# MinghanLi/UniVS

Hardware: AMD Instinct MI355X
Metric: frames/sec per node, 720p T=5 clip, Swin-T 100Q; mask-logit max-abs-err (higher is better)
Workload: dtype f32; 1 GPU; BASELINE config 2: Swin-T UniVS, T=5 @ 720p (736x1280 padded), 100 queries, first clip (no prompt queries); one clip per GPU; frames_per_clip=5, queries=100, parallelism=clip-replicas x1

## Files before the change

univs_amd/build.py:

```python
import os
import shutil
import subprocess
import sys

HERE = os.path.dirname(os.path.abspath(__file__))
CSRC = os.path.join(HERE, "csrc")
LIB = os.path.join(HERE, "libunivs_hip.so")
SOURCES = ["capi.hip", "msda_fwd.hip", "msda_tiled2.hip", "msda_strips.hip", "msda_heads.hip", "msda_bwd.hip", "msda_prepare.hip", "mask_decode.hip", "linear_split.hip", "linear_f16x3.hip", "linear_pair_f16x3.hip", "linear_pair_xres.hip", "gemm_f16x3_stream.hip", "gemm_f16x3_tile.hip", "mlp_f16x3.hip", "small_linear.hip", "cross_attn.hip", "window_attn.hip", "window_attn_f16.hip", "window_attn_qkv.hip", "resample.hip", "semantic_extract.hip", "layer_norm.hip", "group_norm.hip", "softmax.hip", "proca_attn.hip", "prompt_sampler.hip", "transpose.hip", "mask_stats.hip", "image_post.hip", "video_post.hip", "pair_count.hip", "vss_count.hip", "davis_count.hip", "vis_overlap.hip", "pvos_count.hip", "semantic_decode.hip", "frame_resize.hip", "mask_prompt_resize.hip", "png_deflate.hip"]
HEADERS = [os.path.join(CSRC, "common.h"), os.path.join(CSRC, "msda_common.h"), os.path.join(CSRC, "msda_geometry.h"), os.path.join(CSRC, "msda_dev.h"), os.path.join(CSRC, "msda_window_geom.h"), os.path.join(CSRC, "msda_strips_geom.h"), os.path.join(CSRC, "msda_heads_geom.h"), os.path.join(CSRC, "config.h"), os.path.join(CSRC, "window_attn.h"), os.path.join(CSRC, "f16x3.h"), os.path.join(CSRC, "f16x3_kstep.h"), os.path.join(CSRC, "gemm_plan.h"), os.path.join(CSRC, "pair_xres_plan.h"), os.path.join(CSRC, "resample_taps.h"),
           os.path.join(CSRC, "mask_post.h"), os.path.join(CSRC, "count_core.h"), os.path.join(CSRC, "launchers.h"), os.path.join(CSRC, "xattn_merge.h"), os.path.join(CSRC, "skinny_gemm_f32.h"), os.path.join(HERE, "..", "include", "univs_hip.h"),
           os.path.join(HERE, "..", "include", "univs_eval_hip.h"), os.path.join(HERE, "..", "include", "univs_fused_hip.h"),
           os.path.join(HERE, "..", "include", "univs_pvos_hip.h"), os.path.join(HERE, "..", "include", "univs_semantic_hip.h"),
           os.path.join(HERE, "..", "include", "univs_encoder_hip.h"), os.path.join(HERE, "..", "include", "univs_swin_hip.h"),
           os.path.join(HERE, "..", "include", "univs_frames_hip.h"), os.path.join(HERE, "..", "include", "univs_prompts_hip.h"),
           os.path.join(HERE, "..", "include", "univs_png_hip.h")]


def _hipcc():
    for c in (os.environ.get("HIPCC"), shutil.which("hipcc"), "/opt/rocm/bin/hipcc"):
        if c and os.path.exists(c):
            return c
    raise RuntimeError("hipcc not found (set HIPCC or install ROCm)")


def needs_build():
    if not os.path.exists(LIB):
        return True
    t = os.path.getmtime(LIB)
    deps = [os.path.join(CSRC, s) for s in SOURCES if os.path.exists(os.path.join(CSRC, s))] + HEADERS
    return any(os.path.getmtime(d) > t for d in deps)


def _flags(defines=()):
    return ["--offload-arch=gfx950", "-O3", "-std=c++17", "-fPIC", "-fno-gpu-rdc", "-Wall", "-Wno-unused-function",
            "-I", os.path.join(HERE, "..", "include"), *[f"-D{d}" for d in defines]]


def build(force=False, verbose=True, lib=LIB, defines=(), tag=""):
    if not force and not defines and not needs_build():
        return lib
    from concurrent.futures import ThreadPoolExecutor
    objdir = os.path.join(HERE, "_obj" + tag)
    os.makedirs(objdir, exist_ok=True)
    hipcc = _hipcc()
    hdr_t = max(os.path.getmtime(h) for h in HEADERS)
    srcs = [s for s in SOURCES if os.path.exists(os.path.join(CSRC, s))]

    def compile_one(s):
        src, obj = os.path.join(CSRC, s), os.path.join(objdir, s.replace(".hip", ".o"))
        if not force and os.path.exists(obj) and os.path.getmtime(obj) > max(os.path.getmtime(src), hdr_t):
            return obj
        cmd = [hipcc, *_flags(defines), "-c", src, "-o", obj]
        if verbose:
            print("[univs_amd.build]", " ".join(cmd), file=sys.stderr, flush=True)
        subprocess.run(cmd, check=True)
        return obj

    with ThreadPoolExecutor(max_workers=min(8, os.cpu_count() or 2)) as ex:
        objs = list(ex.map(compile_one, srcs))
    cmd = [hipcc, "--offload-arch=gfx950", "-fPIC", "-shared", "-fno-gpu-rdc", *objs, "-o", lib + ".tmp"]
    if verbose:
        print("[univs_amd.build]", " ".join(cmd), file=sys.stderr, flush=True)
    subprocess.run(cmd, check=True)
    os.replace(lib + ".tmp", lib)
    return lib


ABLATIONS = {"plainsplit": ("UNIVS_SPLIT_PLAIN",), "nosplit": ("UNIVS_ABLATE_NOSPLIT",), "nomfma": ("UNIVS_ABLATE_NOMFMA",),
             "nosplit_nomfma": ("UNIVS_ABLATE_NOSPLIT", "UNIVS_ABLATE_NOMFMA"), "trace": ("UNIVS_TRACE_GEMM",), "vtpad8": ("UNIVS_WH_VT_PAD=8", "UNIVS_XA_VS=40"), "gs256": ("UNIVS_GS_THREADS=256",),
             "trace_nosplit_nomfma": ("UNIVS_TRACE_GEMM", "UNIVS_ABLATE_NOSPLIT", "UNIVS_ABLATE_NOMFMA"),
             "heads_nostream": ("S6_ABLATE=1",), "heads_norows": ("S6_ABLATE=2",), "heads_noreduce": ("S6_ABLATE=4",),
             "heads_norecords": ("S6_ABLATE=8",), "heads_nostream_norows": ("S6_ABLATE=3",), "heads_onlyrows": ("S6_ABLATE=13",),
             "heads_skeleton": ("S6_ABLATE=15",), "heads_trace": ("S6_TRACE",),
             "mlp_regstage": ("UNIVS_MLP_REGSTAGE",), "mlp_trace": ("UNIVS_TRACE_MLP",),
             "mlp_trace_nomfma": ("UNIVS_TRACE_MLP", "ML_PS_ABL=1"), "mlp_trace_noreads": ("UNIVS_TRACE_MLP", "ML_PS_ABL=2")}


def build_ablation(name, verbose=False):
    lib = os.path.join(HERE, f"libunivs_hip_{name}.so")
    return build(force=False, verbose=verbose, lib=lib, defines=ABLATIONS[name], tag="_" + name)


if __name__ == "__main__":
    if "--ablate" in sys.argv:
        print(build_ablation(sys.argv[sys.argv.index("--ablate") + 1]))
    else:
        build(force="--force" in sys.argv)
        print(LIB)
```

univs_amd/csrc/gemm_f16x3_stream.hip:

```cpp
#include "common.h"
#include "config.h"
#include "f16x3_kstep.h"
#include "gemm_plan.h"
#include "launchers.h"

#include <algorithm>
#include <cstdlib>

namespace univs {

#ifdef UNIVS_TRACE_GEMM
UNIVS_GT_DECL(g_gs_trace);
#endif
enum { GS_EPI_NONE = EPI_NONE, GS_EPI_RELU = EPI_RELU, GS_EPI_GELU = EPI_GELU, GS_EPI_RESIDUAL = EPI_RESIDUAL };

__global__ __launch_bounds__(256) void presplit_f16x3_kernel(const float* __restrict__ W, int N, int K, int conv_cin, int kperm,
                                                             u32x4* __restrict__ Wp, float* __restrict__ winv) {
  __shared__ unsigned smax;
  const int r = blockIdx.x;
  if (threadIdx.x == 0) smax = 0u;
  __syncthreads();
  const float* src = W + (size_t)r * K;
  auto elem = [&](int k) __attribute__((always_inline)) -> float {
    if (conv_cin == 0) return src[k];
    const int tap = k / conv_cin, ci = k - tap * conv_cin;
    return src[ci * 9 + tap];
  };
  unsigned mx = 0u;
  for (int k = threadIdx.x; k < K; k += blockDim.x) mx = max(mx, __builtin_bit_cast(unsigned, fabsf(elem(k))));
  atomicMax(&smax, mx);
  __syncthreads();
  float s, inv;
  l3_scale(smax, 14, s, inv);
  if (threadIdx.x == 0) winv[r] = inv;
  for (int kc = threadIdx.x; kc < (K >> 3); kc += blockDim.x) {
    f32x4 v0, v1;
#pragma unroll
    for (int e = 0; e < 4; ++e) {
      const int k0 = kperm ? (kc >> 2) * 32 + 4 * (kc & 3) + e : kc * 8 + e;
      v0[e] = elem(k0);
      v1[e] = elem(kperm ? k0 + 16 : k0 + 4);
    }
    f16x8 h, m;
    l3_split8(v0, v1, s, h, m);
    Wp[(size_t)(kc * 2) * N + r] = __builtin_bit_cast(u32x4, h);
    Wp[(size_t)(kc * 2 + 1) * N + r] = __builtin_bit_cast(u32x4, m);
  }
}

int presplit_f16x3(const float* w, int N, int K, int conv_cin, int kperm, void* wp, float* winv, hipStream_t st) {
  if (N <= 0) return UNIVS_OK;
  hipLaunchKernelGGL(presplit_f16x3_kernel, dim3(N), dim3(256), 0, st, w, N, K, conv_cin, kperm, reinterpret_cast<u32x4*>(wp), winv);
  return check_launch("presplit_f16x3");
}

struct GsArgs {
  const float* X;
  const u32x4* Wp;
  const float* winv;
  const float* bias;
  const float* Res;
  float* Y;
  int M, N, K, rows_per_pass, epi;
  int Cin, Cout, H, Wd, HW;
  int tap0;
  int remap;
  const float* affine;
};

template <int RB, int RING, int XMODE, bool AFF = false>
__global__ __launch_bounds__(GS_THREADS, 512 / GS_THREADS) void gemm_f16x3_stream(const GsArgs a) {
  extern __shared__ __attribute__((aligned(16))) u32x4 Wst[];
  [[maybe_unused]] const int gts = UNIVS_GT_SLOT();
  UNIVS_GT(g_gs_trace, gts, 0);
  UNIVS_GT_REAL(g_gs_trace, gts, 62);
  constexpr int Rp = 16 * RB;
  constexpr int SLAB = RING * 4 * 2 * Rp;
  unsigned bx = blockIdx.x, by = blockIdx.y;
  if (a.remap && gridDim.y > 1) {
    const unsigned lw = xcd_remap(blockIdx.x + gridDim.x * blockIdx.y, gridDim.x * gridDim.y);
    bx = lw / gridDim.y;
    by = lw - bx * gridDim.y;
  }
  const int n0 = by * a.rows_per_pass;
  const int R = min(a.rows_per_pass, a.N - n0);
  const int tid = threadIdx.x, lane = tid & 63;
  const int wave = __builtin_amdgcn_readfirstlane(tid >> 6);
  const int M = a.M, N = a.N, K = a.K, epi = a.epi;
  const int KS = K >> 5, KG = KS / RING;
  const int j = lane & 15, g = lane >> 4;
  float* bias_lds = reinterpret_cast<float*>(Wst + 2 * SLAB);
  float* winv_lds = bias_lds + Rp;
  [[maybe_unused]] float* aff_lds = winv_lds + Rp;
  constexpr int NWV = GS_THREADS / 64;

  const int WT = (M + GS_TILE_M - 1) / GS_TILE_M;
  const int wg0 = (int)((long long)WT * bx / gridDim.x), wg1 = (int)((long long)WT * (bx + 1) / gridDim.x);
  const int rounds = (wg1 - wg0 + NWV - 1) / NWV;
  if (rounds == 0) return;

  for (int r = tid; r < Rp; r += GS_THREADS) {
    bias_lds[r] = (a.bias && r < R) ? a.bias[n0 + r] : 0.f;
    winv_lds[r] = r < R ? a.winv[n0 + r] : 0.f;
  }

  constexpr int UNITS = RING * 8 * Rp;
  constexpr int UPT = (UNITS + GS_THREADS - 1) / GS_THREADS;
  constexpr int UPS = (UPT + RING - 1) / RING;
  u32x4 wreg[UPS];
  auto w_fetch = [&](int q, int u) __attribute__((always_inline)) {
#pragma unroll
    for (int v = 0; v < UPS; ++v) {
      const int i = tid + GS_THREADS * (u * UPS + v);
      const int run = i / Rp, rr = i - run * Rp;
      wreg[v] = (u32x4){0u, 0u, 0u, 0u};
      if (u * UPS + v < UPT && i < UNITS && rr < R) wreg[v] = a.Wp[(size_t)(q * RING * 8 + run) * N + n0 + rr];
    }
  };
  auto w_commit = [&](int buf, int u) __attribute__((always_inline)) {
#pragma unroll
    for (int v = 0; v < UPS; ++v) {
      const int i = tid + GS_THREADS * (u * UPS + v);
      if (u * UPS + v < UPT && i < UNITS) Wst[buf * SLAB + i] = wreg[v];
    }
  };
#pragma unroll
  for (int u = 0; u < RING; ++u) {
    w_fetch(0, u);
    w_commit(0, u);
  }

  const long long xbytes = XMODE == 0 ? (long long)M * K * 4 : (long long)(M / a.HW) * a.Cin * a.HW * 4;
  const __amdgpu_buffer_rsrc_t xrs = __builtin_amdgcn_make_buffer_rsrc(const_cast<float*>(a.X), 0, (int)xbytes, 0x00020000);
  const long long ybytes = XMODE == 0 ? (long long)M * N * 4 : (long long)(M / a.HW) * a.Cout * a.HW * 4;
  const __amdgpu_buffer_rsrc_t yrs = __builtin_amdgcn_make_buffer_rsrc(a.Y, 0, (int)ybytes, 0x00020000);
  const __amdgpu_buffer_rsrc_t rrs =
      __builtin_amdgcn_make_buffer_rsrc(const_cast<float*>(epi == GS_EPI_RESIDUAL ? a.Res : a.X), 0, (int)ybytes, 0x00020000);

  struct TileRows {
    unsigned vo[2];
    int py[2], px[2];
    unsigned ao[2];
  };
  auto tile_rows = [&](int tt, TileRows& t) __attribute__((always_inline)) {
#pragma unroll
    for (int c = 0; c < 2; ++c) {
      const int m = min(tt * GS_TILE_M + 16 * c + j, M - 1);
      if (XMODE == 0) {
        t.vo[c] = ((unsigned)m * (unsigned)K + (unsigned)(8 * g)) * 4u;
        t.py[c] = t.px[c] = 0;
        t.ao[c] = 0u;
      } else if (XMODE == 2) {
        const int f = m / a.HW, rem = m - f * a.HW;
        t.py[c] = AFF ? 0 : rem / a.Wd;
        t.px[c] = AFF ? 0 : rem - t.py[c] * a.Wd;
        t.vo[c] = ((unsigned)m * (unsigned)a.Cin + (unsigned)(8 * g)) * 4u;
        t.ao[c] = (unsigned)(((f & 1) * a.Cin + 8 * g) * 8);
      } else {
        const int f = m / a.HW, rem = m - f * a.HW;
        t.py[c] = AFF ? 0 : rem / a.Wd;
        t.px[c] = AFF ? 0 : rem - t.py[c] * a.Wd;
        t.vo[c] = (unsigned)((f * a.Cin + 8 * g) * a.HW + rem) * 4u;
        t.ao[c] = (unsigned)(((f & 1) * a.Cin + 8 * g) * 8);
      }
    }
  };
  f32x4 raw[RING][2][2];
  const int kspt = XMODE != 0 ? a.Cin >> 5 : 1;
  auto load_x = [&](f32x4 (&buf)[2][2], const TileRows& t, int ks) __attribute__((always_inline)) {
    if (XMODE == 0) {
#pragma unroll
      for (int c = 0; c < 2; ++c) {
        buf[c][0] = __builtin_bit_cast(f32x4, __builtin_amdgcn_raw_buffer_load_b128(xrs, t.vo[c], ks * 128, 0));
        buf[c][1] = __builtin_bit_cast(f32x4, __builtin_amdgcn_raw_buffer_load_b128(xrs, t.vo[c] + 16u, ks * 128, 0));
      }
    } else if (XMODE == 2) {
      const int tap_ = ks / kspt, cb = (ks - tap_ * kspt) * 32;
      const int tap = tap_ + a.tap0;
      const int dy = tap / 3 - 1, dx = tap - (tap / 3) * 3 - 1;
#pragma unroll
      for (int c = 0; c < 2; ++c) {
        const bool inb = AFF || ((unsigned)(t.py[c] + dy) < (unsigned)a.H && (unsigned)(t.px[c] + dx) < (unsigned)a.Wd);
        const unsigned vo = inb ? t.vo[c] + (unsigned)((dy * a.Wd + dx) * a.Cin * 4) : 0xFFFFFFE0u;
        buf[c][0] = __builtin_bit_cast(f32x4, __builtin_amdgcn_raw_buffer_load_b128(xrs, vo, cb * 4, 0));
        buf[c][1] = __builtin_bit_cast(f32x4, __builtin_amdgcn_raw_buffer_load_b128(xrs, vo + 16u, cb * 4, 0));
      }
    } else {
      const int tap_ = ks / kspt, cb = (ks - tap_ * kspt) * 32;
      const int tap = tap_ + a.tap0;
      const int dy = tap / 3 - 1, dx = tap - (tap / 3) * 3 - 1;
#pragma unroll
      for (int c = 0; c < 2; ++c) {
        const bool inb = AFF || ((unsigned)(t.py[c] + dy) < (unsigned)a.H && (unsigned)(t.px[c] + dx) < (unsigned)a.Wd);
        const unsigned vo = inb ? t.vo[c] + (unsigned)((dy * a.Wd + dx) * 4) : 0xFFFFFFF0u;
#pragma unroll
        for (int e = 0; e < 8; ++e)
          buf[c][e >> 2][e & 3] = __builtin_bit_cast(float, __builtin_amdgcn_raw_buffer_load_b32(xrs, vo, (cb + e) * a.HW * 4, 0));
      }
    }
  };

  f32x4 acc[RB][2];
  int eset[2];
  float sx[2], sx_inv[2];
  using KS_ = KStep<RB>;
  constexpr int NB = KS_::NB;
  typename KS_::Batch afr[2];
  const unsigned a_lane = KS_::lane(g, j);
  auto read_batch = l3_batch_reader<RB>();

  TileRows t_cur, t_next;
  tile_rows(wg0 + wave, t_cur);
  tile_rows(wg0 + min(1, rounds - 1) * NWV + wave, t_next);
#pragma unroll
  for (int u = 0; u < RING; ++u) load_x(raw[u], t_cur, u);

  UNIVS_GT(g_gs_trace, gts, 2);
  UNIVS_GT_VAL(g_gs_trace, gts, 63, rounds);
  int gq = 0;
  [[maybe_unused]] int aff_f0 = -1, aff_f1 = -1;
#pragma unroll 1
  for (int rd = 0; rd < rounds; ++rd) {
    const int tt = wg0 + rd * NWV + wave;
    const bool tile_ok = tt < wg1;
    if constexpr (AFF) {
      const int r0 = min((wg0 + rd * NWV) * GS_TILE_M, M - 1), r1 = min(r0 + NWV * GS_TILE_M - 1, M - 1);
      const int f0 = r0 / a.HW, f1 = r1 / a.HW;
      if (f0 != aff_f0 || f1 != aff_f1) {
        __syncthreads();
        const int n = (f1 - f0 + 1) * a.Cin;
        for (int i = tid; i < n; i += GS_THREADS) {
          const int f = i < a.Cin ? f0 : f1, ch = i < a.Cin ? i : i - a.Cin;
          *reinterpret_cast<float2*>(aff_lds + ((f & 1) * a.Cin + ch) * 2) = *reinterpret_cast<const float2*>(a.affine + ((size_t)f * a.Cin + ch) * 2);
        }
        aff_f0 = f0;
        aff_f1 = f1;
      }
    }
#pragma unroll
    for (int rb = 0; rb < RB; ++rb) acc[rb][0] = acc[rb][1] = (f32x4){0.f, 0.f, 0.f, 0.f};
    l3_row_scale_reset(eset, sx, sx_inv);
#pragma unroll 1
    for (int q = 0; q < KG; ++q, ++gq) {
      __syncthreads();
      const int bufc = gq & 1, qn = (q + 1 == KG) ? 0 : q + 1;
      const bool last_group = q + 1 == KG;
      const unsigned a_buf = a_lane + (unsigned)(bufc * SLAB * 16);
      read_batch(afr[0], a_buf, std::integral_constant<int, 0>{});
#pragma unroll
      for (int u = 0; u < RING; ++u) {
        if (u > 0) w_commit(bufc ^ 1, u - 1);
        if constexpr (AFF) {
          const unsigned kb = (unsigned)((q * RING + u) * 32 * 8);
#pragma unroll
          for (int c = 0; c < 2; ++c) {
            const f32x4* ap = reinterpret_cast<const f32x4*>(reinterpret_cast<const char*>(aff_lds) + t_cur.ao[c] + kb);
#pragma unroll
            for (int h = 0; h < 2; ++h) {
              const f32x4 p0 = ap[2 * h], p1 = ap[2 * h + 1];
              raw[u][c][h][0] = fmaxf(fma_single(raw[u][c][h][0], p0[0], p0[1]), 0.f);
              raw[u][c][h][1] = fmaxf(fma_single(raw[u][c][h][1], p0[2], p0[3]), 0.f);
              raw[u][c][h][2] = fmaxf(fma_single(raw[u][c][h][2], p1[0], p1[1]), 0.f);
              raw[u][c][h][3] = fmaxf(fma_single(raw[u][c][h][3], p1[2], p1[3]), 0.f);
            }
            __builtin_amdgcn_sched_barrier(0);
          }
        }
        int enew[2];
        if (__builtin_amdgcn_ballot_w64(l3_row_scale_need(raw[u], eset, enew)) != 0) {
#pragma unroll
          for (int c = 0; c < 2; ++c) {
            const bool mine = enew[c] > eset[c] + 2;
            const int en = mine ? enew[c] : eset[c];
            const float ratio = __builtin_bit_cast(float, (unsigned)(127 + max(eset[c] - en, -126)) << 23);
#pragma unroll
            for (int rb = 0; rb < RB; ++rb) acc[rb][c] *= ratio;
            eset[c] = en;
            sx[c] = __builtin_bit_cast(float, (unsigned)(127 + 12 - en) << 23);
            sx_inv[c] = __builtin_bit_cast(float, (unsigned)(127 - 12 + en) << 23);
          }
        }
        float s0 = sx[0], s1 = sx[1];
        asm volatile("" : "+v"(s0), "+v"(s1) : : "memory");
        f16x8 bh[2], bm[2];
        l3_split8(raw[u][0][0], raw[u][0][1], s0, bh[0], bm[0]);
        l3_split8(raw[u][1][0], raw[u][1][1], s1, bh[1], bm[1]);
        __builtin_amdgcn_sched_barrier(0);
        w_fetch(qn, u);
        if (last_group) load_x(raw[u], t_next, u);
        else load_x(raw[u], t_cur, q * RING + u + RING);
        __builtin_amdgcn_sched_barrier(0);
        l3_static_for<0, NB>([&](auto bc) __attribute__((always_inline)) {
          constexpr int b = decltype(bc)::value;
          l3_wait_batch(afr[b & 1]);
          if constexpr (b + 1 < NB) read_batch(afr[(b + 1) & 1], a_buf + (unsigned)u * KS_::kstep, std::integral_constant<int, b + 1>{});
          else if (u + 1 < RING) read_batch(afr[0], a_buf + (unsigned)(u + 1) * KS_::kstep, std::integral_constant<int, 0>{});
          __builtin_amdgcn_sched_barrier(0);
          l3_mfma_batch<RB, b>(afr[b & 1], bh, bm, acc);
          __builtin_amdgcn_sched_barrier(0);
        });
      }
      w_commit(bufc ^ 1, RING - 1);
    }
    UNIVS_GT(g_gs_trace, gts, 3 + 2 * rd);
#pragma unroll
    for (int c = 0; c < 2; ++c) {
      const int m = tt * GS_TILE_M + 16 * c + j;
      const bool row_ok = tile_ok && m < M;
      int fr = 0, rem = 0;
      if (XMODE != 0) {
        fr = min(m, M - 1) / a.HW;
        rem = min(m, M - 1) - fr * a.HW;
      }
      constexpr int RBAT = RB > 4 ? (RB + 1) / 2 : RB;
      [[maybe_unused]] f32x4 resv[RBAT];
      auto load_res = [&](int rb0) __attribute__((always_inline)) {
        if (XMODE == 0 && epi == GS_EPI_RESIDUAL) {
#pragma unroll
          for (int q = 0; q < RBAT; ++q) {
            const int f = min(rb0 + q, RB - 1) * 16 + 4 * g;
            const unsigned off = ((unsigned)m * (unsigned)N + (unsigned)(n0 + f)) * 4u;
            resv[q] = __builtin_bit_cast(f32x4, __builtin_amdgcn_raw_buffer_load_b128(rrs, (row_ok && f < R) ? off : 0xFFFFFFF0u, 0, 0));
          }
        } else {
#pragma unroll
          for (int q = 0; q < RBAT; ++q) resv[q] = (f32x4){0.f, 0.f, 0.f, 0.f};
        }
      };
#pragma unroll
      for (int rb = 0; rb < RB; ++rb) {
        if (rb % RBAT == 0) load_res(rb);
        const int f = rb * 16 + 4 * g;
        const f32x4 wi = *reinterpret_cast<const f32x4*>(winv_lds + f);
        const f32x4 bi = *reinterpret_cast<const f32x4*>(bias_lds + f);
        f32x4 v = (acc[rb][c] * sx_inv[c]) * wi + bi;
        if (XMODE == 0) {
          const unsigned off = ((unsigned)m * (unsigned)N + (unsigned)(n0 + f)) * 4u;
          const unsigned offc = (row_ok && f < R) ? off : 0xFFFFFFF0u;
          if (epi == GS_EPI_RELU) v = __builtin_elementwise_maximum(v, (f32x4){0.f, 0.f, 0.f, 0.f})   ;
          if (epi == GS_EPI_GELU) {
#pragma unroll
            for (int e = 0; e < 4; ++e) v[e] = l3_gelu(v[e]);
          }
          if (epi == GS_EPI_RESIDUAL) v += resv[rb % RBAT];
          __builtin_amdgcn_raw_buffer_store_b128(__builtin_bit_cast(u32x4, v), yrs, offc, 0, 0);
        } else {
          const unsigned off0 = (row_ok && f < R) ? (unsigned)((fr * a.Cout + n0 + f) * a.HW + rem) * 4u
                                                  : 0xFFFFFFF0u - 3u * (unsigned)a.HW * 4u;
          float vx = v.x, vy = v.y, vz = v.z, vw = v.w;
          asm volatile("" : "+v"(vx), "+v"(vy), "+v"(vz), "+v"(vw));
          __builtin_amdgcn_raw_buffer_store_b32(__builtin_bit_cast(unsigned, vx), yrs, off0, 0, 0);
          __builtin_amdgcn_raw_buffer_store_b32(__builtin_bit_cast(unsigned, vy), yrs, off0 + (unsigned)a.HW * 4u, 0, 0);
          __builtin_amdgcn_raw_buffer_store_b32(__builtin_bit_cast(unsigned, vz), yrs, off0 + 2u * (unsigned)a.HW * 4u, 0, 0);
          __builtin_amdgcn_raw_buffer_store_b32(__builtin_bit_cast(unsigned, vw), yrs, off0 + 3u * (unsigned)a.HW * 4u, 0, 0);
        }
      }
    }
    UNIVS_GT(g_gs_trace, gts, 4 + 2 * rd);
    t_cur = t_next;
    tile_rows(wg0 + min(rd + 2, rounds - 1) * NWV + wave, t_next);
  }
  UNIVS_GT_REAL(g_gs_trace, gts, 61);
}

template <int XMODE, bool AFF = false>
static int gs_launch(const GsArgs& a0, hipStream_t st) {
  GsArgs a = a0;
  const StreamPlan p = plan_stream(XMODE, a.M, a.N, a.K, cu_count(), config());
  a.rows_per_pass = p.rows_per_pass;
  a.remap = p.remap;
  const int RB = p.RB, ring = p.ring;
  const size_t lds = p.lds + (AFF ? gs_affine_lds(a.Cin) : 0);
  if (AFF && !stream_affine_plan_covered(RB, ring)) return UNIVS_ERR_NOT_IMPLEMENTED;
  dim3 grid(p.gx, p.passes), block(GS_THREADS);
#define UNIVS_GS(rb, rg)                                                                                          \
  do {                                                                                                            \
    if constexpr (!AFF || stream_affine_plan_covered(rb, rg)) {                                                   \
      (void)hipFuncSetAttribute(reinterpret_cast<const void*>(&gemm_f16x3_stream<rb, rg, XMODE, AFF>),            \
                                hipFuncAttributeMaxDynamicSharedMemorySize, (int)lds);                            \
      hipLaunchKernelGGL((gemm_f16x3_stream<rb, rg, XMODE, AFF>), grid, block, lds, st, a);                       \
    }                                                                                                             \
  } while (0)
#define UNIVS_GS_RB(rb)                    \
  case rb:                                 \
    if (ring == 4) { UNIVS_GS(rb, 4); }    \
    else { UNIVS_GS(rb, 3); }              \
    break
  switch (RB) {
    UNIVS_GS_RB(1);
    UNIVS_GS_RB(2);
    UNIVS_GS_RB(3);
    UNIVS_GS_RB(4);
    UNIVS_GS_RB(5);
    UNIVS_GS_RB(6);
    UNIVS_GS_RB(7);
    default: UNIVS_GS_RB(8);
  }
#undef UNIVS_GS_RB
#undef UNIVS_GS
  return check_launch("gemm_f16x3_stream");
}

int linear_f16x3_stream_f32(const float* x, const void* wp, const float* winv, const float* bias, const float* residual, float* y,
                            long long M, int N, int K, int epi, hipStream_t st) {
  if (M <= 0 || N <= 0) return UNIVS_OK;
  if (!epi_consistent(epi, EPI_RESIDUAL, residual != nullptr) || !stream_linear_covered(M, N, K) ||
      !aligned16(x, wp, y, residual, bias, winv))
    return UNIVS_ERR_NOT_IMPLEMENTED;
  GsArgs a{};
  a.X = x; a.Wp = reinterpret_cast<const u32x4*>(wp); a.winv = winv; a.bias = bias; a.Res = residual; a.Y = y;
  a.M = (int)M; a.N = N; a.K = K; a.epi = epi;
  return gs_launch<0>(a, st);
}

template <int XMODE>
static int gs_conv(const float* x, const void* wp, const float* winv, const float* bias, float* y, int T, int Cin, int Cout, int H, int W,
                   int taps, hipStream_t st, const float* affine = nullptr) {
  if (T <= 0 || Cout <= 0 || H <= 0 || W <= 0) return UNIVS_OK;
  const long long M = (long long)T * H * W;
  if (!stream_conv_covered(M, Cin, Cout, taps) || !aligned16(x, wp, y, winv, bias)) return UNIVS_ERR_NOT_IMPLEMENTED;
  if (affine && (taps != 1 || !stream_affine_covered((long long)H * W, Cin) || (reinterpret_cast<uintptr_t>(affine) & 7)))
    return UNIVS_ERR_NOT_IMPLEMENTED;
  GsArgs a{};
  a.X = x; a.Wp = reinterpret_cast<const u32x4*>(wp); a.winv = winv; a.bias = bias; a.Res = nullptr; a.Y = y;
  a.M = (int)M; a.N = Cout; a.K = taps * Cin; a.epi = GS_EPI_NONE;
  a.Cin = Cin; a.Cout = Cout; a.H = H; a.Wd = W; a.HW = H * W;
  a.tap0 = taps == 9 ? 0 : 4;
  a.affine = affine;
  return affine ? gs_launch<XMODE, true>(a, st) : gs_launch<XMODE>(a, st);
}

int conv3x3_f16x3_f32(const float* x, const void* wp, const float* winv, float* y, int T, int Cin, int Cout, int H, int W,
                      hipStream_t st) {
  return gs_conv<1>(x, wp, winv, nullptr, y, T, Cin, Cout, H, W, 9, st);
}

int conv3x3_nhwc_f16x3_f32(const float* x, const void* wp, const float* winv, float* y, int T, int Cin, int Cout, int H, int W,
                           hipStream_t st) {
  return gs_conv<2>(x, wp, winv, nullptr, y, T, Cin, Cout, H, W, 9, st);
}

int conv1x1_f16x3_f32(const float* x, const void* wp, const float* winv, const float* bias, float* y, int T, int Cin, int Cout, int H,
                      int W, hipStream_t st) {
  return gs_conv<1>(x, wp, winv, bias, y, T, Cin, Cout, H, W, 1, st);
}

int conv1x1_fused_f16x3_f32(const float* x, int channels_last, const float* affine, const void* wp, const float* winv, const float* bias,
                            float* y, int T, int Cin, int Cout, int H, int W, hipStream_t st) {
  return channels_last ? gs_conv<2>(x, wp, winv, bias, y, T, Cin, Cout, H, W, 1, st, affine)
                       : gs_conv<1>(x, wp, winv, bias, y, T, Cin, Cout, H, W, 1, st, affine);
}

}

#ifdef UNIVS_TRACE_GEMM
extern "C" int univs_debug_gemm_trace_stream(unsigned long long* out, int clear) {
  if (clear) {
    static unsigned long long zeros[UNIVS_GT_SLOTS * UNIVS_GT_STAMPS] = {};
    return (int)hipMemcpyToSymbol(HIP_SYMBOL(univs::g_gs_trace), zeros, sizeof(zeros));
  }
  (void)hipDeviceSynchronize();
  return (int)hipMemcpyFromSymbol(out, HIP_SYMBOL(univs::g_gs_trace), sizeof(unsigned long long) * UNIVS_GT_SLOTS * UNIVS_GT_STAMPS);
}
#endif
```

univs_amd/csrc/launchers.h:

```cpp
#pragma once
#include "common.h"

namespace univs {

int msda_forward_generic_f32(const float* value, const LevelTable& lv, const float* loc,
                             const float* attn, int N, int S, int M, int D, int L, int Lq, int P,
                             float* out, hipStream_t st);
int msda_forward_generic_f64(const double* value, const LevelTable& lv, const double* loc,
                             const double* attn, int N, int S, int M, int D, int L, int Lq, int P,
                             double* out, hipStream_t st);

int msda_forward_tiled2_f32(const float* value, const LevelTable& lv, const float* loc, const float* attn, int N,
                            int S, int M, int D, int L, int Lq, int P, float* out, hipStream_t st);

int msda_forward_strips_f32(const float* vhm, const LevelTable& lv, const float* qhm, const float* ref,
                            long long ref_batch_stride, int N, int S, int M, int D, int L, int Lq, int P, float* out,
                            hipStream_t st);

int msda_forward_heads_f32(const float* vhm, const LevelTable& lv, const float* qhm, const float* ref,
                           long long ref_batch_stride, int N, int S, int M, int D, int L, int Lq, int P, float* out,
                           hipStream_t st);

int msda_backward_f32(const float* value, const LevelTable& lv, const float* loc, const float* attn,
                      const float* grad_out, int N, int S, int M, int D, int L, int Lq, int P, float* grad_value,
                      float* grad_loc, float* grad_attn, hipStream_t st);

int msda_prepare_f32(const float* qp, int row_stride, int n_off, const float* ref, long long ref_batch_stride,
                     const LevelTable& lv, int N, int Lq, int M, int L, int P, float* loc, float* attn, hipStream_t st);

int mask_decode_f32(const float* mask_embed, const float* mask_features, int T, int Q, int C,
                    long long HW, float* out, hipStream_t st);
int mask_decode_last_impl();
int mask_decode_attn_f32(const float* mask_embed, const float* feat_lowres, int T, int Q, int C,
                         long long hw, uint8_t* attn_mask, unsigned* row_any_ws, unsigned generation, hipStream_t st);
int attn_mask_rows_reset(uint8_t* attn_mask, const unsigned* row_flags, unsigned generation, long long rows, long long hw, hipStream_t st);

int linear_split_f32(const float* x, const float* w, const float* bias, const float* residual, float* y, long long M, int N,
                     int K, int epi, hipStream_t st, int blk_rows = 0, int blk_cols = 0, const float* winv = nullptr);

int linear_f16x3_f32(const float* x, const float* w, const float* bias, const float* residual, float* y, long long M, int N,
                     int K, int epi, hipStream_t st, int blk_rows, int blk_cols, const float* winv, int n_cu);

int linear_pair_f16x3_f32(const float* x, const float* add, long long add_rows, const void* wp_a, const float* winv_a, const float* bias_a,
                          int N_a, int blk_cols_a, float* y_a, const void* wp_b, const float* winv_b, const float* bias_b, int N_b,
                          int blk_cols_b, float* y_b, long long M, int K, long long blk_rows, hipStream_t st);

int conv3x3_nhwc_f16x3_f32(const float* x, const void* wp, const float* winv, float* y, int T, int Cin, int Cout, int H, int W,
                           hipStream_t st);
int presplit_f16x3(const float* w, int N, int K, int conv_cin, int kperm, void* wp, float* winv, hipStream_t st);
int linear_f16x3_stream_f32(const float* x, const void* wp, const float* winv, const float* bias, const float* residual, float* y,
                            long long M, int N, int K, int epi, hipStream_t st);
int conv3x3_f16x3_f32(const float* x, const void* wp, const float* winv, float* y, int T, int Cin, int Cout, int H, int W,
                      hipStream_t st);
int conv1x1_f16x3_f32(const float* x, const void* wp, const float* winv, const float* bias, float* y, int T, int Cin, int Cout, int H,
                      int W, hipStream_t st);
int conv1x1_fused_f16x3_f32(const float* x, int channels_last, const float* affine, const void* wp, const float* winv, const float* bias,
                            float* y, int T, int Cin, int Cout, int H, int W, hipStream_t st);

int linear_f16x3_tile_f32(const float* x, const void* wp, const float* winv, const float* bias, const float* residual, float* y,
                          long long M, int N, int K, int epi, hipStream_t st);

int mlp_f16x3_f32(const float* x, const void* w1p, const float* w1inv, const float* b1, const void* w2p, const float* w2inv,
                  const float* b2, const float* residual, const float* ln_w, const float* ln_b, float ln_eps, const float* pln_w,
                  const float* pln_b, float pln_eps, const float* post_add, long long post_add_rows, float* y2, float* y, long long M,
                  int C, int Hd, int act, int flags, hipStream_t st);

int small_chain_f32(const float* x, int stages, const void* const* wp, const float* const* winv, const float* const* bias, const int* relu,
                    const float* in_g, const float* in_b, float in_eps, float* xn, float* y, long long M, int out_T, hipStream_t st);
int small_linear_f32(const float* x, const float* xadd, const void* wp, const float* winv, const float* bias, int n_w, int f_off,
                     const float* residual, const float* ln_g, const float* ln_b, float ln_eps, float* y, long long M, int N, int K,
                     int relu, int add_features, int out_T, hipStream_t st);
int small_linear_merged_f32(const float* ws, int plan, int L, int Nb, int Hh, const void* wp, const float* winv, const float* bias, int n_w,
                            int f_off, const float* residual, const float* ln_g, const float* ln_b, float ln_eps, float* y, int N,
                            hipStream_t st);

int cross_attention_f32(const float* q, const float* k, const float* v, const unsigned char* mask, const unsigned* row_flags,
                        unsigned generation, int L, int S, int N, int H, int hd, int ldq, int ldk, int ldv, float scale, float* ws,
                        float* out, hipStream_t st);
int cross_attention_partials_f32(const float* q, const float* k, const float* v, const unsigned char* mask, const unsigned* row_flags,
                                 unsigned generation, int L, int S, int N, int H, int hd, int ldq, int ldk, int ldv, float scale, float* ws,
                                 int* plan_out, hipStream_t st);
size_t cross_attention_workspace_floats(int L, int S, int N, int H);

int window_attention_image_f32(const float* qkv, const float* qkv_bias, const float* bias, const float* shift_mask,
                               int B, int H, int W, int ws, int shift, int nH, int hd, float scale, float* out,
                               hipStream_t st);
int window_attention_f32(const float* qkv, const float* bias, const float* shift_mask, int B_, int nW,
                         int Ntok, int nH, int hd, float scale, float* out, hipStream_t st);

int window_attention_image_f16mma(const float* qkv, const float* qkv_bias, const float* bias, const float* shift_mask, int B,
                                  int H, int W, int ws, int shift, int nH, int hd, float scale, int terms, float* out,
                                  hipStream_t st);

int window_attention_qkv_f16x3(const float* x, const void* wp, const float* winv, const float* qkv_bias, const float* bias,
                               const float* shift_mask, int B, int H, int W, int ws, int shift, int nH, int C, float scale, float* out,
                               hipStream_t st);

int bilinear_resample_f32(const float* in, const float* addend, float* out, long long planes, int Hin, int Win,
                          int Hout, int Wout, hipStream_t st);
int upsample2x_add_f32(const float* in, const float* addend, const float* affine, float* out, long long planes, int Hin, int Win,
                       hipStream_t st);
int normalize_pad_f32(const float* in, float* out, long long T, int C, int H, int W, int Hp, int Wp, const float* mean, const float* stdv,
                      hipStream_t st);
int bilinear_pyramid3_f32(const float* in, float* out2, float* out4, float* out8, long long planes, int H, int W, hipStream_t st);

int bilinear_crop_nearest_f32(const float* in, float* out, int C, int h, int w, int Hp, int Wp, int Hi, int Wi, int hc, int wc, int t_first,
                              int t_step, int K, hipStream_t st);

int layer_norm_f32(const float* x, const float* res, const float* gamma, const float* beta, long long rows, int C,
                   float eps, float* sum_out, float* out, const float* addend, float* out2, long long addend_rows, hipStream_t st);
int patch_merge_norm_f32(const float* x, const float* gamma, const float* beta, int B, int H, int W, int C, float eps, float* out,
                         hipStream_t st);

int group_norm_affine_f32(const float* x, const float* gamma, const float* beta, int N, int C, long long HW, int groups, float eps,
                          float* ws, long long ws_floats, float* affine, hipStream_t st);
int group_norm_f32(const float* x, const float* gamma, const float* beta, int N, int C, long long HW, int groups,
                   float eps, int relu, float* ws, long long ws_floats, float* out, hipStream_t st);

int masked_softmax_f32(float* scores, const unsigned char* mask, int N, int h, int L, int S, hipStream_t st);

int proca_attention_f32(const float* qkv0, const float* kd, const float* vd, int Qp, int L, int T, int h, int hd, float scale,
                        float* out, hipStream_t st);

int prompt_prefix_f32(const float* masks, const float* boxes, int Fk, int n, int h, int w, int scale, float feat_thresh,
                      float* feat_masks, unsigned* stats, uint8_t* sel, int* rowcnt, uint8_t* fmb, int* counts, uint8_t* valid,
                      uint8_t* visible, hipStream_t st);
int prompt_draw(const uint8_t* sel, const int* rowcnt, const uint8_t* fmb, const int* counts, const float* u, const float* keys,
                const long long* tab, int Fk, int n, int h, int w, int HW, int R, long long* point_idx, long long* dense_idx,
                uint8_t* empty, float* point_coords, hipStream_t st);
int prompt_point_pe_f32(const float* xy, const float* z, const float* dim_t, const float* dim_tz, float scale, int Fk, int n, int F,
                        float* out, hipStream_t st);
int token_mean_f32(const float* x, const float* add, int n, int L, int T, int C, float* out, hipStream_t st);
int prompt_tokens_f32(const float* feats, const long long* fs, const float* pos, const long long* ps, const float* qfeat,
                      const float* qpe, const long long* dense_idx, const uint8_t* empty, const uint8_t* valid, const float* boxes,
                      const long long* kf, int Fk, int n, int R, int T, int C, int h_img, int w_img, float* fd, float* pd, uint8_t* attn,
                      hipStream_t st);

int transpose_f32(const float* in, float* out, long long B, int R, int C, long long in_bstride, long long out_bstride,
                  const float* row_affine, const float* addend, float* out2, hipStream_t st);
int decoder_memory_f32(const float* x, const float* level_embed, const float* yx, const float* pos_z, float* mem, float* key, int T, int C,
                       int HW, hipStream_t st);
int patch_embed4_f32(const float* x, const float* w, const float* bias, const float* ln_g, const float* ln_b, float eps, float* out, int T,
                     int H, int W, int E, hipStream_t st);

int mask_stats_f32(const float* x, long long planes, int inner, long long stride_outer, long long stride_inner, int H, int W, int hv, int wv,
                   float t_hi, float t_lo, float t_box, int* out, hipStream_t st);

int image_mask_stats_f32(const float* L, int Q, int h, int w, int Hp, int Wp, int hi, int wi, int* out, hipStream_t st);
int image_panoptic_ids_f32(const float* L, int Q, int h, int w, int Hp, int Wp, int hi, int wi, const int* planes, const float* scores, int K,
                           int* ids, int* counts, hipStream_t st);
int image_panoptic_paint_i32(const int* ids, int hi, int wi, const int* lut, int K, int H0, int W0, int* out, int* seen, hipStream_t st);
int image_semseg_f32(const float* L, int Q, int h, int w, int Hp, int Wp, int hi, int wi, const int* planes, const float* P, int Qs, int C,
                     float* R, hipStream_t st);
int image_instance_masks_u8(const float* L, int Q, int h, int w, int Hp, int Wp, int hi, int wi, const int* planes, int N, int H0, int W0,
                            unsigned char* masks, int* boxes, hipStream_t st);

int minvis_accumulate_f32(float* S, int Q, int V, int h, int w, const float* M, int Qm, int T, const int* perm, int i, hipStream_t st);
int video_mask_stats_f32(const float* M, int Q, int V, int h, int w, int Hp, int Wp, int hi, int wi, const int* rows, int K, int step,
                         int* counts, hipStream_t st);
int video_instance_masks_u8(const float* M, int Q, int V, int h, int w, int Hp, int Wp, int hi, int wi, const int* rows, int N, int H0,
                            int W0, unsigned char* masks, hipStream_t st);
int video_panoptic_ids_i32(const float* M, int Q, int V, int h, int w, int Hp, int Wp, int hi, int wi, const int* rows, const float* scores,
                           int K, int* ids, hipStream_t st);
int video_panoptic_counts_i32(const float* M, int Q, int V, int h, int w, int Hp, int Wp, int hi, int wi, const int* rows, int K,
                              const int* ids, int H0, int W0, int* counts, hipStream_t st);
int video_panoptic_paint_i32(const float* M, int Q, int V, int h, int w, int Hp, int Wp, int hi, int wi, const int* rows, int K,
                             const int* ids, const int* lut, int H0, int W0, int* out, hipStream_t st);

int panoptic_pair_counts(const void* gt, int gt_rgb, const void* pred, int pred_rgb, int T, int H, int W, const int* gt_ids, int G,
                         const int* pred_ids, int P, int* counts, int* first_unknown, hipStream_t st);

int vss_video_counts(const unsigned char* gt, const unsigned char* pred, int T, int H, int W, int C, int* confusion, int* windows,
                     int* overflow, hipStream_t st);

int davis_counts(const unsigned char* gt, const unsigned char* pred, int T, int H, int W, int G, int P, int radius, int use_void,
                 int* region, int* n_gt, int* n_fg, int* match, hipStream_t st);

int vis_overlap_counts(const int* dt_bounds, const int* dt_starts, const int* gt_bounds, const int* gt_ones, const int* gt_starts, int D,
                       int G, int T, int H, int W, int gt_max_bounds, int* inter, hipStream_t st);

int pvos_counts(const unsigned char* gt, const unsigned char* pred, int T, int H, int W, int d, int K, int* counts, hipStream_t st);

int semantic_quality_counts_f32(const float* mask_embed, const float* features, int T, int N, int C, int HW, int t_step, float t_hi,
                                float t_lo, int* counts, hipStream_t st);

int resize_frames_u8(const unsigned char* src, int T, int Hi, int Wi, int Ho, int Wo, const int* first_x, const int* count_x,
                     const int* coef_x, int ksize_x, const int* first_y, const int* count_y, const int* coef_y, int ksize_y, int swap_rb,
                     unsigned char* out, hipStream_t st);

int resize_rle_masks_u8(const int* bounds, const int* starts, long long n_bounds, int N, int H, int W, const int* ty, const int* tx, int Ho,
                        int Wo, unsigned char* masks, int* boxes, hipStream_t st);

int png_deflate_maps(const void* src, int src_is_i32, int N, int H, int W, const unsigned char* lut, int K, int C, int rows_per_stripe,
                     unsigned char* scratch, unsigned char* out, long long* offsets, hipStream_t st);

}
```

Measured before the change: 387.3 frames/s.

## Add wide-Cout 3x3 conv kernel with LDS-streamed weights for Cout=256

Adds a new implicit-GEMM 3x3 convolution kernel specialised for 256 output channels. Each 512-thread workgroup streams split-f16 weight images through a four-slot LDS ring using global_load_lds, and each wave computes a 32-row tile against all 256 outputs with f16x3 MFMA accumulation and persistent rounds. The aim is to reuse weights across eight waves and cut weight traffic compared with the generic streaming conv. Both NCHW and NHWC conv3x3 entry points try it first and fall back when a shape or alignment is not covered. It adds large LDS and register pressure, which may lower occupancy.

Measured after the change: 392.2 frames/s (median of 6 runs). +1.3%, better.

```diff
diff --git a/univs_amd/build.py b/univs_amd/build.py
--- a/univs_amd/build.py
+++ b/univs_amd/build.py
@@ -6,8 +6,8 @@
 HERE = os.path.dirname(os.path.abspath(__file__))
 CSRC = os.path.join(HERE, "csrc")
 LIB = os.path.join(HERE, "libunivs_hip.so")
-SOURCES = ["capi.hip", "msda_fwd.hip", "msda_tiled2.hip", "msda_strips.hip", "msda_heads.hip", "msda_bwd.hip", "msda_prepare.hip", "mask_decode.hip", "linear_split.hip", "linear_f16x3.hip", "linear_pair_f16x3.hip", "linear_pair_xres.hip", "gemm_f16x3_stream.hip", "gemm_f16x3_tile.hip", "mlp_f16x3.hip", "small_linear.hip", "cross_attn.hip", "window_attn.hip", "window_attn_f16.hip", "window_attn_qkv.hip", "resample.hip", "semantic_extract.hip", "layer_norm.hip", "group_norm.hip", "softmax.hip", "proca_attn.hip", "prompt_sampler.hip", "transpose.hip", "mask_stats.hip", "image_post.hip", "video_post.hip", "pair_count.hip", "vss_count.hip", "davis_count.hip", "vis_overlap.hip", "pvos_count.hip", "semantic_decode.hip", "frame_resize.hip", "mask_prompt_resize.hip", "png_deflate.hip"]
-HEADERS = [os.path.join(CSRC, "common.h"), os.path.join(CSRC, "msda_common.h"), os.path.join(CSRC, "msda_geometry.h"), os.path.join(CSRC, "msda_dev.h"), os.path.join(CSRC, "msda_window_geom.h"), os.path.join(CSRC, "msda_strips_geom.h"), os.path.join(CSRC, "msda_heads_geom.h"), os.path.join(CSRC, "config.h"), os.path.join(CSRC, "window_attn.h"), os.path.join(CSRC, "f16x3.h"), os.path.join(CSRC, "f16x3_kstep.h"), os.path.join(CSRC, "gemm_plan.h"), os.path.join(CSRC, "pair_xres_plan.h"), os.path.join(CSRC, "resample_taps.h"),
+SOURCES = ["capi.hip", "msda_fwd.hip", "msda_tiled2.hip", "msda_strips.hip", "msda_heads.hip", "msda_bwd.hip", "msda_prepare.hip", "mask_decode.hip", "linear_split.hip", "linear_f16x3.hip", "linear_pair_f16x3.hip", "linear_pair_xres.hip", "gemm_f16x3_stream.hip", "conv3x3_wide.hip", "gemm_f16x3_tile.hip", "mlp_f16x3.hip", "small_linear.hip", "cross_attn.hip", "window_attn.hip", "window_attn_f16.hip", "window_attn_qkv.hip", "resample.hip", "semantic_extract.hip", "layer_norm.hip", "group_norm.hip", "softmax.hip", "proca_attn.hip", "prompt_sampler.hip", "transpose.hip", "mask_stats.hip", "image_post.hip", "video_post.hip", "pair_count.hip", "vss_count.hip", "davis_count.hip", "vis_overlap.hip", "pvos_count.hip", "semantic_decode.hip", "frame_resize.hip", "mask_prompt_resize.hip", "png_deflate.hip"]
+HEADERS = [os.path.join(CSRC, "common.h"), os.path.join(CSRC, "msda_common.h"), os.path.join(CSRC, "msda_geometry.h"), os.path.join(CSRC, "msda_dev.h"), os.path.join(CSRC, "msda_window_geom.h"), os.path.join(CSRC, "msda_strips_geom.h"), os.path.join(CSRC, "msda_heads_geom.h"), os.path.join(CSRC, "config.h"), os.path.join(CSRC, "window_attn.h"), os.path.join(CSRC, "f16x3.h"), os.path.join(CSRC, "f16x3_kstep.h"), os.path.join(CSRC, "gemm_plan.h"), os.path.join(CSRC, "pair_xres_plan.h"), os.path.join(CSRC, "conv3x3_wide_plan.h"), os.path.join(CSRC, "resample_taps.h"),
            os.path.join(CSRC, "mask_post.h"), os.path.join(CSRC, "count_core.h"), os.path.join(CSRC, "launchers.h"), os.path.join(CSRC, "xattn_merge.h"), os.path.join(CSRC, "skinny_gemm_f32.h"), os.path.join(HERE, "..", "include", "univs_hip.h"),
            os.path.join(HERE, "..", "include", "univs_eval_hip.h"), os.path.join(HERE, "..", "include", "univs_fused_hip.h"),
            os.path.join(HERE, "..", "include", "univs_pvos_hip.h"), os.path.join(HERE, "..", "include", "univs_semantic_hip.h"),
diff --git a/univs_amd/csrc/conv3x3_wide.hip b/univs_amd/csrc/conv3x3_wide.hip
--- /dev/null
+++ b/univs_amd/csrc/conv3x3_wide.hip
@@ -0,0 +1,230 @@
+#include "common.h"
+#include "config.h"
+#include "conv3x3_wide_plan.h"
+#include "f16x3_kstep.h"
+#include "launchers.h"
+
+namespace univs {
+
+struct CwArgs {
+  const float* X;
+  const u32x4* Wp;
+  const float* winv;
+  float* Y;
+  int M, Cin, H, Wd, HW, rounds;
+};
+
+__device__ __forceinline__ void cw_glds16(const u32x4* base, unsigned voff, unsigned lds_dst) {
+  unsigned keep;
+  const unsigned dst = __builtin_amdgcn_readfirstlane(lds_dst);
+  asm volatile("s_mov_b32 %0, m0\n\ts_mov_b32 m0, %3\n\ts_nop 0\n\tglobal_load_lds_dwordx4 %1, %2\n\ts_mov_b32 m0, %0"
+               : "=&s"(keep) : "v"(voff), "s"(base), "s"(dst) : "memory");
+}
+
+template <int XMODE>
+__global__ __launch_bounds__(CW_THREADS) void conv3x3_wide(const CwArgs a) {
+  static_assert(XMODE == 1 || XMODE == 2, "operand layouts");
+  extern __shared__ __attribute__((aligned(16))) u32x4 Lds[];
+  constexpr int RB = CW_COUT / 16;
+  constexpr int IMG = 4 * 2 * CW_COUT;
+  constexpr int NWV = CW_THREADS / 64;
+  constexpr int UPT = IMG / CW_THREADS;
+  constexpr int XL = XMODE == 1 ? 16 : 4;
+  constexpr int NB = RB / 2;
+  static_assert(IMG % CW_THREADS == 0 && CW_IMAGES == 4 && 2 * XL < 64, "stream geometry");
+  const int M = a.M;
+  const int tid = threadIdx.x, lane = tid & 63;
+  const int wave = __builtin_amdgcn_readfirstlane(tid >> 6);
+  const int j = lane & 15, g = lane >> 4;
+  const int kspt = a.Cin >> 5, KS = 9 * kspt;
+  const int WT = (M + CW_TILE_M - 1) / CW_TILE_M;
+  const int rd0 = (int)blockIdx.x * a.rounds;
+  const int rounds = min(a.rounds, (WT + NWV - 1) / NWV - rd0);
+  if (rounds <= 0) return;
+  float* winv_lds = reinterpret_cast<float*>(Lds + CW_IMAGES * IMG);
+  for (int r = tid; r < CW_COUT; r += CW_THREADS) winv_lds[r] = a.winv[r];
+
+  const unsigned lds_base = __builtin_amdgcn_readfirstlane((unsigned)(uintptr_t)Lds);
+  const unsigned w_voff = (unsigned)tid * 16u;
+  auto w_request = [&](int s, int img) __attribute__((always_inline)) {
+    const u32x4* base = a.Wp + (size_t)s * IMG;
+    const unsigned dst = lds_base + (unsigned)((img * IMG + 64 * wave) * 16);
+#pragma unroll
+    for (int v = 0; v < UPT; ++v) cw_glds16(base + CW_THREADS * v, w_voff, dst + (unsigned)(CW_THREADS * v * 16));
+  };
+#pragma unroll
+  for (int s = 0; s < 2; ++s) w_request(s, s);
+
+  const long long xbytes = (long long)(M / a.HW) * a.Cin * a.HW * 4;
+  const __amdgpu_buffer_rsrc_t xrs = __builtin_amdgcn_make_buffer_rsrc(const_cast<float*>(a.X), 0, (int)xbytes, 0x00020000);
+  const long long ybytes = (long long)(M / a.HW) * CW_COUT * a.HW * 4;
+  const __amdgpu_buffer_rsrc_t yrs = __builtin_amdgcn_make_buffer_rsrc(a.Y, 0, (int)ybytes, 0x00020000);
+  struct TileRows {
+    unsigned vo[2];
+    int py[2], px[2];
+  };
+  auto tile_rows = [&](int tt, TileRows& t) __attribute__((always_inline)) {
+#pragma unroll
+    for (int c = 0; c < 2; ++c) {
+      const int m = min(tt * CW_TILE_M + 16 * c + j, M - 1);
+      const int f = m / a.HW, rem = m - f * a.HW;
+      t.py[c] = rem / a.Wd;
+      t.px[c] = rem - t.py[c] * a.Wd;
+      t.vo[c] = XMODE == 2 ? ((unsigned)m * (unsigned)a.Cin + (unsigned)(8 * g)) * 4u
+                           : (unsigned)((f * a.Cin + 8 * g) * a.HW + rem) * 4u;
+    }
+  };
+  auto load_x = [&](f32x4 (&buf)[2][2], const TileRows& t, int tap, int kc) __attribute__((always_inline)) {
+    const int cb = kc * 32;
+    const int dy = tap / 3 - 1, dx = tap - (tap / 3) * 3 - 1;
+#pragma unroll
+    for (int c = 0; c < 2; ++c) {
+      const bool inb = (unsigned)(t.py[c] + dy) < (unsigned)a.H && (unsigned)(t.px[c] + dx) < (unsigned)a.Wd;
+      if (XMODE == 2) {
+        const unsigned vo = inb ? t.vo[c] + (unsigned)((dy * a.Wd + dx) * a.Cin * 4) : 0xFFFFFFE0u;
+        buf[c][0] = __builtin_bit_cast(f32x4, __builtin_amdgcn_raw_buffer_load_b128(xrs, vo, cb * 4, 0));
+        buf[c][1] = __builtin_bit_cast(f32x4, __builtin_amdgcn_raw_buffer_load_b128(xrs, vo + 16u, cb * 4, 0));
+      } else {
+        const unsigned vo = inb ? t.vo[c] + (unsigned)((dy * a.Wd + dx) * 4) : 0xFFFFFFF0u;
+#pragma unroll
+        for (int e = 0; e < 8; ++e)
+          buf[c][e >> 2][e & 3] = __builtin_bit_cast(float, __builtin_amdgcn_raw_buffer_load_b32(xrs, vo, (cb + e) * a.HW * 4, 0));
+      }
+    }
+  };
+
+  typedef u32x4 Batch[2][2];
+  auto read_batch = [](Batch& d, unsigned base, auto bc) __attribute__((always_inline)) {
+    constexpr int b = decltype(bc)::value;
+    u32x4& d00 = d[0][0];
+    u32x4& d01 = d[0][1];
+    u32x4& d10 = d[1][0];
+    u32x4& d11 = d[1][1];
+    asm volatile("ds_read_b128 %0, %4 offset:%5\n\tds_read_b128 %1, %4 offset:%6\n\tds_read_b128 %2, %4 offset:%7\n\tds_read_b128 %3, %4 offset:%8"
+                 : "=&v"(d00), "=&v"(d01), "=&v"(d10), "=&v"(d11)
+                 : "v"(base), "n"(b * 512), "n"(b * 512 + CW_COUT * 16), "n"(b * 512 + 256), "n"(b * 512 + 256 + CW_COUT * 16)
+                 : "memory");
+  };
+  const unsigned a_lane = (unsigned)((g * 2 * CW_COUT + j) * 16);
+
+  f32x4 acc[RB][2];
+  int eset[2];
+  float sx[2], sx_inv[2];
+  Batch afr[2];
+  f32x4 raw[2][2][2];
+
+  TileRows t_ld, t_nx;
+  tile_rows(rd0 * NWV + wave, t_ld);
+  tile_rows((rd0 + min(1, rounds - 1)) * NWV + wave, t_nx);
+  load_x(raw[0], t_ld, 0, 0);
+  load_x(raw[1], t_ld, 0, 1);
+  int ld_tap = 0, ld_kc = 2;
+  int img = 0;
+  int sreq = 2;
+  asm volatile("s_waitcnt vmcnt(0)" ::: "memory");
+
+#pragma unroll 1
+  for (int rd = 0; rd < rounds; ++rd) {
+    const int tt = (rd0 + rd) * NWV + wave;
+#pragma unroll
+    for (int rb = 0; rb < RB; ++rb) acc[rb][0] = acc[rb][1] = (f32x4){0.f, 0.f, 0.f, 0.f};
+    l3_row_scale_reset(eset, sx, sx_inv);
+#pragma unroll 1
+    for (int q = 0; q < KS; q += 2) {
+      l3_static_for<0, 2>([&](auto uc) __attribute__((always_inline)) {
+        constexpr int u = decltype(uc)::value;
+        if constexpr (u == 0) {
+          asm volatile("s_waitcnt vmcnt(%0)" : : "n"(2 * XL) : "memory");
+          __syncthreads();
+          w_request(sreq, (img + 2) & (CW_IMAGES - 1));
+          w_request(sreq + 1, (img + 3) & (CW_IMAGES - 1));
+          sreq = sreq + 2 == KS ? 0 : sreq + 2;
+        }
+        const unsigned a_buf = a_lane + (unsigned)(img * IMG * 16);
+        img = (img + 1) & (CW_IMAGES - 1);
+        read_batch(afr[0], a_buf, std::integral_constant<int, 0>{});
+        int enew[2];
+        if (__builtin_amdgcn_ballot_w64(l3_row_scale_need(raw[u], eset, enew)) != 0) l3_row_scale_lower<RB>(enew, acc, eset, sx, sx_inv);
+        float s0 = sx[0], s1 = sx[1];
+        asm volatile("" : "+v"(s0), "+v"(s1) : : "memory");
+        f16x8 bh[2], bm[2];
+        l3_split8(raw[u][0][0], raw[u][0][1], s0, bh[0], bm[0]);
+        l3_split8(raw[u][1][0], raw[u][1][1], s1, bh[1], bm[1]);
+        __builtin_amdgcn_sched_barrier(0);
+        load_x(raw[u], t_ld, ld_tap, ld_kc);
+        if (++ld_kc == kspt) {
+          ld_kc = 0;
+          if (++ld_tap == 9) {
+            ld_tap = 0;
+            t_ld = t_nx;
+          }
+        }
+        __builtin_amdgcn_sched_barrier(0);
+        l3_static_for<0, NB>([&](auto bc) __attribute__((always_inline)) {
+          constexpr int b = decltype(bc)::value;
+          l3_wait_batch(afr[b & 1]);
+          if constexpr (b + 1 < NB) read_batch(afr[(b + 1) & 1], a_buf, std::integral_constant<int, b + 1>{});
+          __builtin_amdgcn_sched_barrier(0);
+#pragma unroll
+          for (int qb = 0; qb < 2; ++qb) {
+            constexpr int rb0 = 2 * b;
+            const f16x8 ah = __builtin_bit_cast(f16x8, afr[b & 1][qb][0]);
+            const f16x8 am = __builtin_bit_cast(f16x8, afr[b & 1][qb][1]);
+            acc[rb0 + qb][0] = __builtin_amdgcn_mfma_f32_16x16x32_f16(am, bh[0], acc[rb0 + qb][0], 0, 0, 0);
+            acc[rb0 + qb][1] = __builtin_amdgcn_mfma_f32_16x16x32_f16(am, bh[1], acc[rb0 + qb][1], 0, 0, 0);
+            acc[rb0 + qb][0] = __builtin_amdgcn_mfma_f32_16x16x32_f16(ah, bm[0], acc[rb0 + qb][0], 0, 0, 0);
+            acc[rb0 + qb][1] = __builtin_amdgcn_mfma_f32_16x16x32_f16(ah, bm[1], acc[rb0 + qb][1], 0, 0, 0);
+            acc[rb0 + qb][0] = __builtin_amdgcn_mfma_f32_16x16x32_f16(ah, bh[0], acc[rb0 + qb][0], 0, 0, 0);
+            acc[rb0 + qb][1] = __builtin_amdgcn_mfma_f32_16x16x32_f16(ah, bh[1], acc[rb0 + qb][1], 0, 0, 0);
+          }
+          __builtin_amdgcn_sched_barrier(0);
+        });
+      });
+    }
+    const bool tile_ok = tt < WT;
+#pragma unroll
+    for (int c = 0; c < 2; ++c) {
+      const int m = tt * CW_TILE_M + 16 * c + j;
+      const bool row_ok = tile_ok && m < M;
+      const int fr = min(m, M - 1) / a.HW, rem = min(m, M - 1) - fr * a.HW;
+#pragma unroll
+      for (int rb = 0; rb < RB; ++rb) {
+        const int f = rb * 16 + 4 * g;
+        const f32x4 wi = *reinterpret_cast<const f32x4*>(winv_lds + f);
+        const f32x4 v = (acc[rb][c] * sx_inv[c]) * wi + (f32x4){0.f, 0.f, 0.f, 0.f};
+        const unsigned off0 = row_ok ? (unsigned)((fr * CW_COUT + f) * a.HW + rem) * 4u : 0xFFFFFFF0u - 3u * (unsigned)a.HW * 4u;
+        float vx = v.x, vy = v.y, vz = v.z, vw = v.w;
+        asm volatile("" : "+v"(vx), "+v"(vy), "+v"(vz), "+v"(vw));
+        __builtin_amdgcn_raw_buffer_store_b32(__builtin_bit_cast(unsigned, vx), yrs, off0, 0, 0);
+        __builtin_amdgcn_raw_buffer_store_b32(__builtin_bit_cast(unsigned, vy), yrs, off0 + (unsigned)a.HW * 4u, 0, 0);
+        __builtin_amdgcn_raw_buffer_store_b32(__builtin_bit_cast(unsigned, vz), yrs, off0 + 2u * (unsigned)a.HW * 4u, 0, 0);
+        __builtin_amdgcn_raw_buffer_store_b32(__builtin_bit_cast(unsigned, vw), yrs, off0 + 3u * (unsigned)a.HW * 4u, 0, 0);
+      }
+    }
+    tile_rows((rd0 + min(rd + 2, rounds - 1)) * NWV + wave, t_nx);
+  }
+  asm volatile("s_waitcnt vmcnt(0)" ::: "memory");
+}
+
+int conv3x3_wide_f32(int xmode, const float* x, const void* wp, const float* winv, float* y, int T, int Cin, int Cout, int H, int W,
+                     hipStream_t st) {
+  if (config().linear_ablate == CW_ABLATE_OFF || T <= 0 || H <= 0 || W <= 0) return 0;
+  const long long M = (long long)T * H * W;
+  if (!conv3x3_wide_covered(M, Cin, Cout) || !aligned16(x, wp, y, winv)) return 0;
+  const WidePlan p = plan_conv3x3_wide(M, cu_count());
+  CwArgs a;
+  a.X = x; a.Wp = reinterpret_cast<const u32x4*>(wp); a.winv = winv; a.Y = y;
+  a.M = (int)M; a.Cin = Cin; a.H = H; a.Wd = W; a.HW = H * W; a.rounds = p.rounds;
+  const size_t lds = conv3x3_wide_lds();
+  if (xmode == 2) {
+    (void)hipFuncSetAttribute(reinterpret_cast<const void*>(&conv3x3_wide<2>), hipFuncAttributeMaxDynamicSharedMemorySize, (int)lds);
+    hipLaunchKernelGGL((conv3x3_wide<2>), dim3(p.nwg), dim3(CW_THREADS), lds, st, a);
+  } else {
+    (void)hipFuncSetAttribute(reinterpret_cast<const void*>(&conv3x3_wide<1>), hipFuncAttributeMaxDynamicSharedMemorySize, (int)lds);
+    hipLaunchKernelGGL((conv3x3_wide<1>), dim3(p.nwg), dim3(CW_THREADS), lds, st, a);
+  }
+  const int rc = check_launch("conv3x3_wide_f32");
+  return rc == UNIVS_OK ? 1 : rc;
+}
+
+}
diff --git a/univs_amd/csrc/conv3x3_wide_plan.h b/univs_amd/csrc/conv3x3_wide_plan.h
--- /dev/null
+++ b/univs_amd/csrc/conv3x3_wide_plan.h
@@ -0,0 +1,33 @@
+#pragma once
+#include "gemm_plan.h"
+
+namespace univs {
+
+constexpr int CW_THREADS = 512;
+constexpr int CW_TILE_M = 32;
+constexpr int CW_COUT = 256;
+constexpr int CW_IMAGES = 4;
+constexpr int CW_ABLATE_OFF = 12;
+
+constexpr size_t CW_IMAGE_BYTES = (size_t)4 * 2 * CW_COUT * 16;
+inline size_t conv3x3_wide_lds() { return CW_IMAGES * CW_IMAGE_BYTES + (size_t)2 * CW_COUT * 4; }
+
+inline bool conv3x3_wide_covered(long long M, int Cin, int Cout) {
+  return stream_conv_covered(M, Cin, Cout, 9) && Cout == CW_COUT && conv3x3_wide_lds() <= (size_t)RESIDENT_LDS_CAP;
+}
+
+struct WidePlan {
+  unsigned nwg;
+  int rounds;
+};
+inline WidePlan plan_conv3x3_wide(long long M, int n_cu) {
+  constexpr int NWV = CW_THREADS / 64;
+  const long long WT = (M + CW_TILE_M - 1) / CW_TILE_M;
+  const long long total = (WT + NWV - 1) / NWV;
+  WidePlan p;
+  p.rounds = (int)((total + std::max(1, n_cu) - 1) / std::max(1, n_cu));
+  p.nwg = (unsigned)((total + p.rounds - 1) / p.rounds);
+  return p;
+}
+
+}
diff --git a/univs_amd/csrc/gemm_f16x3_stream.hip b/univs_amd/csrc/gemm_f16x3_stream.hip
--- a/univs_amd/csrc/gemm_f16x3_stream.hip
+++ b/univs_amd/csrc/gemm_f16x3_stream.hip
@@ -432,11 +432,13 @@
 
 int conv3x3_f16x3_f32(const float* x, const void* wp, const float* winv, float* y, int T, int Cin, int Cout, int H, int W,
                       hipStream_t st) {
+  if (const int rc = conv3x3_wide_f32(1, x, wp, winv, y, T, Cin, Cout, H, W, st); rc != 0) return rc == 1 ? UNIVS_OK : rc;
   return gs_conv<1>(x, wp, winv, nullptr, y, T, Cin, Cout, H, W, 9, st);
 }
 
 int conv3x3_nhwc_f16x3_f32(const float* x, const void* wp, const float* winv, float* y, int T, int Cin, int Cout, int H, int W,
                            hipStream_t st) {
+  if (const int rc = conv3x3_wide_f32(2, x, wp, winv, y, T, Cin, Cout, H, W, st); rc != 0) return rc == 1 ? UNIVS_OK : rc;
   return gs_conv<2>(x, wp, winv, nullptr, y, T, Cin, Cout, H, W, 9, st);
 }
 
diff --git a/univs_amd/csrc/launchers.h b/univs_amd/csrc/launchers.h
--- a/univs_amd/csrc/launchers.h
+++ b/univs_amd/csrc/launchers.h
@@ -56,6 +56,9 @@
                       int W, hipStream_t st);
 int conv1x1_fused_f16x3_f32(const float* x, int channels_last, const float* affine, const void* wp, const float* winv, const float* bias,
                             float* y, int T, int Cin, int Cout, int H, int W, hipStream_t st);
+
+int conv3x3_wide_f32(int xmode, const float* x, const void* wp, const float* winv, float* y, int T, int Cin, int Cout, int H, int W,
+                     hipStream_t st);
 
 int linear_f16x3_tile_f32(const float* x, const void* wp, const float* winv, const float* bias, const float* residual, float* y,
                           long long M, int N, int K, int epi, hipStream_t st);
```
